# NVlabs/UnseenObjectClustering

Hardware: AMD Instinct MI355X
Metric: frames/sec at 640x480 RGB-D, two-stage clustering (higher is better)
Workload: dtype f32; 1 GPU; configs[3] frames: full two-stage (crop-and-refine) segmentation of single 640x480 RGB-D frames; throughput schedule 3 streams x 4-frame launch sets (one frame at a time: `latency`); frame=640x480, seeds=100, iters=10, crop=224, total_frames=513, frames_per_gpu=513, collective=False, frames_in_flight_per_gpu=12, streams_per_gpu=3, frames_per_launch=4

## Files before the change

### unseenobjectclustering_amd/csrc/meanshift.hip

```cpp
#include "common.h"
#include "prof.h"

#include <limits.h>
#include <math.h>
#include <stdlib.h>

#include <mutex>
#include <type_traits>
#include <utility>

namespace uoc {

constexpr int C = UOC_EMBED_DIM;
constexpr int FPS_THREADS = 256;
constexpr int FPS_MAX_BLOCKS = 1024;
constexpr int HC_THREADS = 256;
constexpr int HC_MAX_BLOCKS = 1024;
constexpr int ZP = 72;
constexpr int NLAB = UOC_MAX_SEEDS;

constexpr int MS_COSINE = UOC_METRIC_COSINE;
constexpr int MS_EUCLIDEAN = UOC_METRIC_EUCLIDEAN;
constexpr float XX_OUT = 1e30f;

struct ArgMax {
  float val;
  int idx;
};

__device__ __forceinline__ bool better(const ArgMax &a, const ArgMax &b) {
  return a.val > b.val || (a.val == b.val && a.idx < b.idx);
}

__device__ __forceinline__ ArgMax wave_argmax(ArgMax v) {
#pragma unroll
  for (int off = 32; off >= 1; off >>= 1) {
    ArgMax o;
    o.val = __shfl_xor(v.val, off);
    o.idx = __shfl_xor(v.idx, off);
    if (better(o, v)) v = o;
  }
  return v;
}

template <int NH, int MET>
__global__ __launch_bounds__(FPS_THREADS) void fps_step_kernel(
    const float *__restrict__ X, int n, int m, int step, int num_init, const int *__restrict__ first_index,
    float *__restrict__ dmin, float *__restrict__ seeds, int *__restrict__ indices,
    const ArgMax *__restrict__ part_in, ArgMax *__restrict__ part_out) {
  const int b = blockIdx.y;
  const int nblk = gridDim.x;
  X += (size_t)b * NH * n * C;
  dmin += (size_t)b * n;
  seeds += (size_t)b * NH * m * C;
  indices += (size_t)b * m;
  part_in += (size_t)b * FPS_MAX_BLOCKS;
  part_out += (size_t)b * FPS_MAX_BLOCKS;

  __shared__ ArgMax red[FPS_THREADS / 64];
  const int tid = threadIdx.x, lane = tid & 63, wave = tid >> 6;

  const bool given = step < num_init;
  int cur;
  if (given) {
    cur = -1;
  } else if (step == 0) {
    cur = first_index[b];
    if (cur < 0 || cur >= n) cur = 0;
  } else {
    ArgMax best = {-INFINITY, INT_MAX};
    for (int i = tid; i < nblk; i += FPS_THREADS) {
      ArgMax a = part_in[i];
      if (better(a, best)) best = a;
    }
    best = wave_argmax(best);
    if (lane == 0) red[wave] = best;
    __syncthreads();
    best = red[0];
#pragma unroll
    for (int w = 1; w < FPS_THREADS / 64; ++w)
      if (better(red[w], best)) best = red[w];
    cur = best.idx;
    if (cur < 0 || cur >= n) cur = 0;
    __syncthreads();
  }
  if (blockIdx.x == 0) {
    if (tid == 0) indices[step] = cur;
    if (!given && tid < NH * C)
      seeds[((size_t)(tid / C) * m + step) * C + tid % C] = X[((size_t)(tid / C) * n + cur) * C + tid % C];
  }
  if (step == m - 1) return;

  const int t = lane & 15, g = lane >> 4;
  float4 sv[NH];
#pragma unroll
  for (int h = 0; h < NH; ++h)
    sv[h] = given ? *reinterpret_cast<const float4 *>(seeds + ((size_t)h * m + step) * C + 4 * t)
                  : *reinterpret_cast<const float4 *>(X + ((size_t)h * n + cur) * C + 4 * t);
  ArgMax best = {-INFINITY, INT_MAX};
  const int nchunk = (n + 63) >> 6;
  for (int chunk = blockIdx.x * (FPS_THREADS / 64) + wave; chunk < nchunk; chunk += nblk * (FPS_THREADS / 64)) {
    const int base = chunk << 6;
    float4 x[NH][16];
#pragma unroll
    for (int h = 0; h < NH; ++h)
#pragma unroll
      for (int i = 0; i < 16; ++i) {
        const int p = base + 4 * i + g;
        x[h][i] = (p < n) ? *reinterpret_cast<const float4 *>(X + ((size_t)h * n + p) * C + 4 * t)
                          : make_float4(0.f, 0.f, 0.f, 0.f);
      }
    float mine = 0.f;
#pragma unroll
    for (int i = 0; i < 16; ++i) {
      float s;
      if constexpr (MET == MS_EUCLIDEAN) {
        s = 0.f;
#pragma unroll
        for (int h = 0; h < NH; ++h) {
          const float dx = x[h][i].x - sv[h].x, dy = x[h][i].y - sv[h].y, dz = x[h][i].z - sv[h].z,
                      dw = x[h][i].w - sv[h].w;
          s = fmaf(dx, dx, s);
          s = fmaf(dy, dy, s);
          s = fmaf(dz, dz, s);
          s = fmaf(dw, dw, s);
        }
      } else {
        s = x[0][i].x * sv[0].x;
        s = fmaf(x[0][i].y, sv[0].y, s);
        s = fmaf(x[0][i].z, sv[0].z, s);
        s = fmaf(x[0][i].w, sv[0].w, s);
#pragma unroll
        for (int h = 1; h < NH; ++h) {
          s = fmaf(x[h][i].x, sv[h].x, s);
          s = fmaf(x[h][i].y, sv[h].y, s);
          s = fmaf(x[h][i].z, sv[h].z, s);
          s = fmaf(x[h][i].w, sv[h].w, s);
        }
      }
      s = row16_sum(s);
      if (t == i) mine = s;
    }
    const int p = base + 4 * t + g;
    if (p < n) {
      float d = MET == MS_EUCLIDEAN ? sqrtf(mine) : 0.5f * (1.0f - mine);
      if (step > 0) d = fminf(d, dmin[p]);
      dmin[p] = d;
      if (d > best.val) {
        best.val = d;
        best.idx = p;
      }
    }
  }
  best = wave_argmax(best);
  if (lane == 0) red[wave] = best;
  __syncthreads();
  if (tid == 0) {
    best = red[0];
#pragma unroll
    for (int w = 1; w < FPS_THREADS / 64; ++w)
      if (better(red[w], best)) best = red[w];
    part_out[blockIdx.x] = best;
  }
}

__device__ int g_fps_timeout = 0;

constexpr int FPP_THREADS = 512;
constexpr int FPP_WAVES = FPP_THREADS / 64;
constexpr int FPP_RS = 3;
constexpr int FPP_LS = 1;
constexpr int FPP_SLOTS = FPP_RS + FPP_LS;
constexpr int FPP_PIX_PER_BLOCK = FPP_THREADS * FPP_SLOTS;

__device__ __forceinline__ ArgMax wave_argmax_fast(ArgMax a) {
  float v = a.val;
  v = fmaxf(v, dpp_f<0xB1>(v));
  v = fmaxf(v, dpp_f<0x4E>(v));
  v = fmaxf(v, dpp_f<0x141>(v));
  v = fmaxf(v, dpp_f<0x140>(v));
  const int vi = __float_as_int(v);
  const float m = fmaxf(fmaxf(__int_as_float(__builtin_amdgcn_readlane(vi, 0)), __int_as_float(__builtin_amdgcn_readlane(vi, 16))),
                        fmaxf(__int_as_float(__builtin_amdgcn_readlane(vi, 32)), __int_as_float(__builtin_amdgcn_readlane(vi, 48))));
  int i = (a.val == m) ? a.idx : INT_MAX;
  i = min(i, dpp_i<0xB1>(i));
  i = min(i, dpp_i<0x4E>(i));
  i = min(i, dpp_i<0x141>(i));
  i = min(i, dpp_i<0x140>(i));
  const int mi = min(min(__builtin_amdgcn_readlane(i, 0), __builtin_amdgcn_readlane(i, 16)),
                     min(__builtin_amdgcn_readlane(i, 32), __builtin_amdgcn_readlane(i, 48)));
  return ArgMax{m, mi};
}

__device__ __forceinline__ unsigned long long fpp_pack(float val, int idx, int tag) {
  return ((unsigned long long)__float_as_uint(val) << 32) | (unsigned)(idx & 0xFFFFFF) | ((unsigned)(tag & 0xFF) << 24);
}

template <int MET>
__global__ __launch_bounds__(FPP_THREADS) void fps_persistent_kernel(
    const float *__restrict__ X, int n, int m, int bpi, int nslots, const int *__restrict__ first_index,
    float *__restrict__ seeds, int *__restrict__ indices, unsigned long long *gran, int *status) {
  extern __shared__ __attribute__((aligned(16))) float smem[];
  __shared__ ArgMax red[FPP_WAVES];
  __shared__ int s_idx;
  const int item = blockIdx.x / bpi, blk = blockIdx.x - item * bpi;
  X += (size_t)item * n * C;
  seeds += (size_t)item * m * C;
  indices += (size_t)item * m;
  const int tid = threadIdx.x, lane = tid & 63, wave = tid >> 6;
  const int pbase = blk * (FPP_THREADS * nslots) + tid;
  float4 *lds = reinterpret_cast<float4 *>(smem) + tid;

  typedef float f32x2 __attribute__((ext_vector_type(2)));
  static_assert(FPP_RS == 3, "pixels 0/1 packed, pixel 2 scalar");
  f32x2 x01[C];
  float x2[C];
#pragma unroll
  for (int j = 0; j < FPP_RS; ++j) {
    const int p = pbase + j * FPP_THREADS;
    const bool ok = j < nslots && p < n;
#pragma unroll
    for (int c4 = 0; c4 < C / 4; ++c4) {
      const float4 v = ok ? *reinterpret_cast<const float4 *>(X + (size_t)p * C + 4 * c4) : make_float4(0.f, 0.f, 0.f, 0.f);
      const float e[4] = {v.x, v.y, v.z, v.w};
#pragma unroll
      for (int k = 0; k < 4; ++k) {
        if (j == 0) x01[4 * c4 + k].x = e[k];
        if (j == 1) x01[4 * c4 + k].y = e[k];
        if (j == 2) x2[4 * c4 + k] = e[k];
      }
    }
  }
  if (nslots > FPP_RS) {
    const int p = pbase + FPP_RS * FPP_THREADS;
#pragma unroll
    for (int c4 = 0; c4 < C / 4; ++c4)
      lds[c4 * FPP_THREADS] = (p < n) ? *reinterpret_cast<const float4 *>(X + (size_t)p * C + 4 * c4)
                                      : make_float4(0.f, 0.f, 0.f, 0.f);
  }
  float dm[FPP_SLOTS];
#pragma unroll
  for (int j = 0; j < FPP_SLOTS; ++j) dm[j] = 0.f;
  float xx[FPP_SLOTS] = {};
  if constexpr (MET == MS_EUCLIDEAN) {
    f32x2 q01 = {0.f, 0.f};
    float q2 = 0.f, q3 = 0.f;
#pragma unroll
    for (int c = 0; c < C; ++c) {
      q01 = __builtin_elementwise_fma(x01[c], x01[c], q01);
      q2 = fmaf(x2[c], x2[c], q2);
    }
    if (nslots > FPP_RS) {
#pragma unroll
      for (int c4 = 0; c4 < C / 4; ++c4) {
        const float4 v = lds[c4 * FPP_THREADS];
        q3 = fmaf(v.x, v.x, q3);
        q3 = fmaf(v.y, v.y, q3);
        q3 = fmaf(v.z, v.z, q3);
        q3 = fmaf(v.w, v.w, q3);
      }
    }
    xx[0] = q01.x;
    xx[1] = q01.y;
    xx[2] = q2;
    xx[3] = q3;
  }

  int cur = __builtin_amdgcn_readfirstlane(first_index[item]);
  if (cur < 0 || cur >= n) cur = 0;
  if (blk == 0) {
    if (tid == 0) indices[0] = cur;
    if (tid < 16) *reinterpret_cast<float4 *>(seeds + 4 * tid) = *reinterpret_cast<const float4 *>(X + (size_t)cur * C + 4 * tid);
  }
#ifdef UOC_FPS_TIMING
  unsigned long long tc_comp = 0, tc_red = 0, tc_sweep = 0, tc_tail = 0;
#define UOC_T(v) const unsigned long long v = __builtin_amdgcn_s_memtime()
#else
#define UOC_T(v)
#endif
  for (int step = 0; step + 1 < m; ++step) {
    UOC_T(t1_);
    const float *__restrict__ srow = X + (size_t)cur * C;
    ArgMax best = {-INFINITY, INT_MAX};
    f32x2 s01 = {0.f, 0.f};
#pragma unroll
    for (int c = 0; c < C; ++c) s01 = __builtin_elementwise_fma(x01[c], f32x2{srow[c], srow[c]}, s01);
    float ss = 0.f;
    if constexpr (MET == MS_EUCLIDEAN) {
#pragma unroll
      for (int c = 0; c < C; ++c) ss = fmaf(srow[c], srow[c], ss);
    }
    auto dist = [&](float s_, float xx_) {
      if constexpr (MET == MS_EUCLIDEAN) return sqrtf(fmaxf(fmaf(-2.0f, s_, xx_ + ss), 0.0f));
      else return 0.5f * (1.0f - s_);
    };
    float s2 = 0.f;
    if (nslots > 2) {
#pragma unroll
      for (int c = 0; c < C; ++c) s2 = fmaf(x2[c], srow[c], s2);
    }
#pragma unroll
    for (int j = 0; j < FPP_RS; ++j) {
      if (j < nslots) {
        const float s_ = j == 0 ? s01.x : j == 1 ? s01.y : s2;
        float d_ = dist(s_, xx[j]);
        if (step > 0) d_ = fminf(d_, dm[j]);
        dm[j] = d_;
        const int p_ = pbase + j * FPP_THREADS;
        if (p_ < n && d_ > best.val) {
          best.val = d_;
          best.idx = p_;
        }
      }
    }
    if (nslots > FPP_RS) {
      float s_ = 0.f;
#pragma unroll
      for (int c4 = 0; c4 < C / 4; ++c4) {
        const float4 v = lds[c4 * FPP_THREADS];
        s_ = fmaf(v.x, srow[4 * c4 + 0], s_);
        s_ = fmaf(v.y, srow[4 * c4 + 1], s_);
        s_ = fmaf(v.z, srow[4 * c4 + 2], s_);
        s_ = fmaf(v.w, srow[4 * c4 + 3], s_);
      }
      float d_ = dist(s_, xx[FPP_RS]);
      if (step > 0) d_ = fminf(d_, dm[FPP_RS]);
      dm[FPP_RS] = d_;
      const int p_ = pbase + FPP_RS * FPP_THREADS;
      if (p_ < n && d_ > best.val) {
        best.val = d_;
        best.idx = p_;
      }
    }
    UOC_T(t2_);
    best = wave_argmax_fast(best);
    if (lane == 0) red[wave] = best;
    __syncthreads();
    UOC_T(t3_);
    if (wave == 0) {
      ArgMax b2 = lane < FPP_WAVES ? red[lane] : ArgMax{-INFINITY, INT_MAX};
      b2 = wave_argmax_fast(b2);
      unsigned long long *row = gran + ((size_t)(step & 1) * gridDim.x + (size_t)item * bpi);
      const int tag = (step + 1) & 0xFF;
      if (lane == 0) __hip_atomic_store(row + blk, fpp_pack(b2.val, b2.idx, tag), __ATOMIC_RELAXED, __HIP_MEMORY_SCOPE_AGENT);
      ArgMax acc = {-INFINITY, INT_MAX};
      unsigned spins = 0;
      bool done = false;
      while (!done) {
        bool ok = true;
        ArgMax a = {-INFINITY, INT_MAX};
        unsigned long long gv[4];
#pragma unroll
        for (int k = 0; k < 4; ++k)
          gv[k] = (lane + 64 * k < bpi) ? __hip_atomic_load(row + lane + 64 * k, __ATOMIC_RELAXED, __HIP_MEMORY_SCOPE_AGENT)
                                        : ((unsigned long long)tag << 24);
#pragma unroll
        for (int k = 0; k < 4; ++k) {
          const unsigned long long v = gv[k];
          ok &= (int)((v >> 24) & 0xFF) == tag;
          if (lane + 64 * k < bpi) {
            ArgMax c = {__uint_as_float((unsigned)(v >> 32)), (int)(v & 0xFFFFFF)};
            if (better(c, a)) a = c;
          }
        }
        if (__all(ok)) {
          acc = a;
          done = true;
        } else {
          __builtin_amdgcn_s_sleep(1);
          if (++spins > (1u << 22) || (((spins & 1023) == 0) && __hip_atomic_load(status, __ATOMIC_RELAXED, __HIP_MEMORY_SCOPE_AGENT))) {
            if (lane == 0) {
              __hip_atomic_store(status, 1, __ATOMIC_RELAXED, __HIP_MEMORY_SCOPE_AGENT);
              __hip_atomic_store(&g_fps_timeout, 1, __ATOMIC_RELAXED, __HIP_MEMORY_SCOPE_AGENT);
            }
            acc = ArgMax{0.f, 0};
            done = true;
          }
        }
      }
      acc = wave_argmax_fast(acc);
      if (lane == 0) s_idx = acc.idx;
    }
    __syncthreads();
    UOC_T(t4_);
    cur = __builtin_amdgcn_readfirstlane(s_idx);
    if (cur < 0 || cur >= n) cur = 0;
    if (blk == 0) {
      if (tid == 0) indices[step + 1] = cur;
      if (tid < 16)
        *reinterpret_cast<float4 *>(seeds + (size_t)(step + 1) * C + 4 * tid) =
            *reinterpret_cast<const float4 *>(X + (size_t)cur * C + 4 * tid);
    }
#ifdef UOC_FPS_TIMING
    const unsigned long long t5_ = __builtin_amdgcn_s_memtime();
    tc_comp += t2_ - t1_;
    tc_red += t3_ - t2_;
    tc_sweep += t4_ - t3_;
    tc_tail += t5_ - t4_;
#endif
  }
#ifdef UOC_FPS_TIMING
  if ((blockIdx.x == 0 || blockIdx.x == gridDim.x / 2) && tid == 0)
    printf("[fps timing blk %d] per step (cycles): compute %.1f reduce %.1f sweep %.1f tail %.1f\n", (int)blockIdx.x,
           tc_comp / (double)(m - 1), tc_red / (double)(m - 1), tc_sweep / (double)(m - 1), tc_tail / (double)(m - 1));
#endif
#undef UOC_T
}

__device__ __forceinline__ float f4c(const float4 &v, int e) { return e == 0 ? v.x : e == 1 ? v.y : e == 2 ? v.z : v.w; }
__device__ __forceinline__ f32x4 mfma4(float a, float b, f32x4 c) {
  return __builtin_amdgcn_mfma_f32_16x16x4f32(a, b, c, 0, 0, 0);
}

template <int ST, int NH>
__device__ __forceinline__ void lds_stage_seeds(const float *Z, int m, int tid, float *Zs) {
  for (int i = tid; i < NH * ST * 16 * (C / 4); i += HC_THREADS) {
    const int h = i / (ST * 16 * (C / 4)), j = i % (ST * 16 * (C / 4));
    const int row = j / (C / 4), c4 = j % (C / 4);
    float4 v = make_float4(0.f, 0.f, 0.f, 0.f);
    if (row < m) v = *reinterpret_cast<const float4 *>(Z + ((size_t)h * m + row) * C + 4 * c4);
    *reinterpret_cast<float4 *>(Zs + (h * ST * 16 + row) * ZP + 4 * c4) = v;
  }
}
template <int ST, int NH>
__device__ __forceinline__ void lds_seed_norms(const float *Zs, int tid, float *zzs) {
  if (tid < ST * 16) {
    float p = 0.f;
    for (int h = 0; h < NH; ++h)
      for (int c = 0; c < C; ++c) {
        const float z = Zs[(h * ST * 16 + tid) * ZP + c];
        p = fmaf(z, z, p);
      }
    zzs[tid] = p;
  }
}
template <int NH>
__device__ __forceinline__ void lds_pixel_norms(const float4 (&xa)[NH * 4], int q, float (&xx)[4]) {
  float p = 0.f;
#pragma unroll
  for (int v = 0; v < NH * 4; ++v) {
    p = fmaf(xa[v].x, xa[v].x, p);
    p = fmaf(xa[v].y, xa[v].y, p);
    p = fmaf(xa[v].z, xa[v].z, p);
    p = fmaf(xa[v].w, xa[v].w, p);
  }
  p += __shfl_xor(p, 16);
  p += __shfl_xor(p, 32);
#pragma unroll
  for (int r = 0; r < 4; ++r) xx[r] = __shfl(p, 4 * q + r);
}

template <int ST, int NH, int MET>
__global__ __launch_bounds__(HC_THREADS) __attribute__((amdgpu_waves_per_eu(2))) void hc_iter_kernel(const float *__restrict__ X, int n,
                                                             const float *__restrict__ Z, int m, float kappa,
                                                             float *__restrict__ partial_, int nvb) {
  static_assert(NH == 2, "64-d fields run hc_iter_flat_kernel");
  extern __shared__ __attribute__((aligned(16))) float smem[];
  constexpr bool EUC = MET == MS_EUCLIDEAN;
  __shared__ float zzs[EUC ? ST * 16 : 1];
  __shared__ float wred[EUC ? 4 * ST * 16 : 1];
  float *Zs = smem;
  const int b = blockIdx.y;
  const int nblk = nvb;
  const int hz = blockIdx.z;
  X += (size_t)b * NH * n * C;
  Z += (size_t)b * NH * m * C;

  const int tid = threadIdx.x, lane = tid & 63, wave = tid >> 6;
  const int t = lane & 15, q = lane >> 4;
  float *const wpartial = partial_ + (size_t)gridDim.y * nblk * NH * (ST * 16) * C;
  for (int vb = blockIdx.x; vb < nvb; vb += gridDim.x) {
  float *partial = partial_ + (((size_t)b * nblk + vb) * NH + hz) * (ST * 16) * C;

  lds_stage_seeds<ST, NH>(Z, m, tid, Zs);
  __syncthreads();
  float ws[ST];
  if constexpr (EUC) {
    lds_seed_norms<ST, NH>(Zs, tid, zzs);
#pragma unroll
    for (int s = 0; s < ST; ++s) ws[s] = 0.f;
    __syncthreads();
  }

  f32x4 acc[ST][4];
#pragma unroll
  for (int s = 0; s < ST; ++s)
#pragma unroll
    for (int ct = 0; ct < 4; ++ct) acc[s][ct] = f32x4{0.f, 0.f, 0.f, 0.f};

  const int ntile = (n + 15) >> 4;
  const int stride = nblk * (HC_THREADS / 64);
  int tile = vb * (HC_THREADS / 64) + wave;

  float4 xa[NH * 4], xb[4];
  auto load_tile = [&](int tl, float4(&a)[NH * 4], float4(&bb)[4]) {
    const int pa = tl * 16 + t;
#pragma unroll
    for (int v = 0; v < NH * 4; ++v)
      a[v] = (tl < ntile && pa < n)
                 ? *reinterpret_cast<const float4 *>(X + ((size_t)(v >> 2) * n + pa) * C + 16 * (v & 3) + 4 * q)
                 : make_float4(0.f, 0.f, 0.f, 0.f);
#pragma unroll
    for (int r = 0; r < 4; ++r) {
      const int pb = tl * 16 + 4 * q + r;
      bb[r] = (tl < ntile && pb < n) ? *reinterpret_cast<const float4 *>(X + ((size_t)hz * n + pb) * C + 4 * t)
                                     : make_float4(0.f, 0.f, 0.f, 0.f);
    }
  };
  load_tile(tile, xa, xb);

  for (; tile < ntile; tile += stride) {
    f32x4 Sv[ST];
    float wv[ST][4];
    int zo = 0;
    asm volatile("" : "+v"(zo));
    const float *Zt = Zs + zo;
    float xx[4];
    if constexpr (EUC) {
      lds_pixel_norms<NH>(xa, q, xx);
#pragma unroll
      for (int r = 0; r < 4; ++r)
        if (tile * 16 + 4 * q + r >= n) xx[r] = XX_OUT;
    }
#pragma unroll
    for (int i = 0; i < ST + 2; ++i) {
      if (i >= 1 && i - 1 < ST) {
        if constexpr (EUC) {
          const float zz = zzs[16 * (i - 1) + t];
#pragma unroll
          for (int r = 0; r < 4; ++r)
            wv[i - 1][r] = expf(-kappa * fmaxf(fmaf(-2.0f, Sv[i - 1][r], zz + xx[r]), 0.0f));
          ws[i - 1] += (wv[i - 1][0] + wv[i - 1][1]) + (wv[i - 1][2] + wv[i - 1][3]);
        } else {
#pragma unroll
          for (int r = 0; r < 4; ++r) wv[i - 1][r] = expf(kappa * Sv[i - 1][r]);
        }
      }
      if (i < ST) Sv[i] = f32x4{0.f, 0.f, 0.f, 0.f};
      if (i < ST) {
#pragma unroll
        for (int k = 0; k < 16; ++k) {
          const int v = k >> 2, e = k & 3;
          const float4 zb = *reinterpret_cast<const float4 *>(Zt + (ST * 16 + 16 * i + t) * ZP + 16 * v + 4 * q);
          Sv[i] = mfma4(f4c(xa[4 + v], e), f4c(zb, e), Sv[i]);
        }
      }
#pragma unroll
      for (int k = 0; k < 16; ++k) {
        if (i < ST) {
          const int v = k >> 2, e = k & 3;
          const float4 zb = *reinterpret_cast<const float4 *>(Zt + (16 * i + t) * ZP + 16 * v + 4 * q);
          Sv[i] = mfma4(f4c(xa[v], e), f4c(zb, e), Sv[i]);
        }
        if (i >= 2) {
          const int r = k >> 2, ct = k & 3;
          acc[i - 2][ct] = mfma4(wv[i - 2][r], f4c(xb[r], ct), acc[i - 2][ct]);
        }
      }
    }
// ... 949 lines not shown
  ArgMax *part[2];
  float *hc_partial;
  int *counts;
  int *num_unique;
  int *seed_labels;
  float *Z;
  int hc_nblk;
  int nh;
  size_t total;
};

static int hc_virtual_blocks(int n) {
  const int ntile = (n + 15) / 16;
  const int tiles_per_wave = 16;
  int nvb = (ntile + 4 * tiles_per_wave - 1) / (4 * tiles_per_wave);
  if (nvb > 256) nvb = 256;
  if (nvb < 1) nvb = 1;
  return nvb;
}

static int hc_physical_blocks(int batch, int nvb, int per_cu) {
  const int slots = (device_num_cu() > 0 ? device_num_cu() : 256) * per_cu;
  int best = 1;
  long best_cost = -1;
  for (int p = 1; p <= nvb; ++p) {
    const long rounds = ((long)p * batch + slots - 1) / slots;
    const long cost = rounds * ((nvb + p - 1) / p);
    if (best_cost < 0 || cost < best_cost) {
      best_cost = cost;
      best = p;
    }
  }
  return best;
}

static int hc_blocks(int batch, int n) {
  const int ntile = (n + 15) / 16;
  int nblk = 512 / (batch > 0 ? batch : 1);
  if (nblk < 8) nblk = 8;
  const int maxb = (ntile + 3) / 4;
  if (nblk > maxb) nblk = maxb;
  if (nblk > HC_MAX_BLOCKS) nblk = HC_MAX_BLOCKS;
  if (nblk < 1) nblk = 1;
  return nblk;
}

static MsWorkspace carve(void *base, int batch, int n, int nh = 1) {
  MsWorkspace w;
  size_t off = 0;
  auto take = [&](size_t bytes) {
    void *p = base ? (void *)((char *)base + off) : nullptr;
    off += align_up(bytes, 256);
    return p;
  };
  w.hc_nblk = hc_virtual_blocks(n);
  w.dmin = (float *)take((size_t)batch * n * sizeof(float));
  w.part[0] = (ArgMax *)take((size_t)batch * FPS_MAX_BLOCKS * sizeof(ArgMax));
  w.part[1] = (ArgMax *)take((size_t)batch * FPS_MAX_BLOCKS * sizeof(ArgMax));
  w.hc_partial = (float *)take((size_t)batch * w.hc_nblk * (nh * NLAB * C + NLAB) * sizeof(float));
  w.counts = (int *)take((size_t)batch * NLAB * sizeof(int));
  w.num_unique = (int *)take((size_t)batch * sizeof(int));
  w.seed_labels = (int *)take((size_t)batch * NLAB * sizeof(int));
  w.Z = (float *)take((size_t)batch * nh * NLAB * C * sizeof(float));
  w.nh = nh;
  w.total = off;
  return w;
}

static int check_common(const void *X, int batch, int n, int m, void *ws, size_t ws_bytes, int nh = 1) {
  UOC_REQUIRE(X != nullptr, "X is null");
  UOC_REQUIRE(batch >= 1 && batch <= 65535, "batch=%d out of range [1,65535]", batch);
  UOC_REQUIRE(n >= 1, "n=%d must be >= 1", n);
  UOC_REQUIRE(m >= 1 && m <= UOC_MAX_SEEDS, "num_seeds=%d out of range [1,%d]", m, UOC_MAX_SEEDS);
  UOC_REQUIRE(((uintptr_t)X & 15) == 0, "X must be 16-byte aligned");
  const size_t need = carve(nullptr, batch, n, nh).total;
  UOC_REQUIRE(ws != nullptr && ws_bytes >= need, "workspace too small: %zu < %zu", ws_bytes, need);
  UOC_REQUIRE(((uintptr_t)ws & 255) == 0, "workspace must be 256-byte aligned");
  return UOC_OK;
}

static int fps_blocks(int n) {
  const int nchunk = (n + 63) / 64;
  int nblk = (nchunk + 3) / 4;
  if (nblk > FPS_MAX_BLOCKS) nblk = FPS_MAX_BLOCKS;
  if (nblk < 1) nblk = 1;
  return nblk;
}

static int g_fps_persistent = -1;
static std::atomic<int> g_fps_fallbacks{0};
static std::atomic<int> g_fps_stream_ordering{0};
static int fps_persistent_plan(int batch, int n, int *bpi, int *nslots) {
  const int g_num_cu = device_num_cu();
  if (g_num_cu <= 0) return 0;
  if (g_fps_persistent < 0) {
    const char *e = getenv("UOC_FPS_PERSISTENT");
    g_fps_persistent = e ? atoi(e) : 1;
  }
  if (!g_fps_persistent || n >= (1 << 24)) return 0;
  int b = g_num_cu / batch;
  if (b < 1) return 0;
  if (b > 256) b = 256;
  const int per_block = (n + b - 1) / b;
  int ns = (per_block + FPP_THREADS - 1) / FPP_THREADS;
  if (ns > FPP_SLOTS) return 0;
  if (ns < 1) ns = 1;
  const int pack = FPP_SLOTS;
  if (pack > ns) ns = pack < FPP_SLOTS ? pack : FPP_SLOTS;
  b = (n + FPP_THREADS * ns - 1) / (FPP_THREADS * ns);
  *bpi = b;
  *nslots = ns;
  return 1;
}

template <int... Vs, class F>
static void dispatch(int v, F &&f) {
  (void)((v == Vs && (f(std::integral_constant<int, Vs>{}), true)) || ...);
}
template <class F>
static void dispatch_metric_halves(int met, int nh, F &&f) {
  dispatch<MS_COSINE, MS_EUCLIDEAN>(met, [&](auto MET) { dispatch<1, 2>(nh, [&](auto NH) { f(MET, NH); }); });
}
template <class F>
static void dispatch_shape(int met, int nh, int m, F &&f) {
  dispatch_metric_halves(met, nh, [&](auto MET, auto NH) {
    dispatch<1, 2, 3, 4, 5, 6, 7, 8>((m + 15) / 16, [&](auto ST) { f(ST, NH, MET); });
  });
}

static int run_select_seeds_streaming(const float *X, int batch, int n, int m, const int32_t *first, float *seeds,
                                      int32_t *indices, const MsWorkspace &w, hipStream_t st, int num_init = 0,
                                      int met = MS_COSINE);

struct FpsChain {
  std::mutex mu;
  hipEvent_t ev[kMaxDevices] = {};
  hipEvent_t event() {
    const int d = current_device();
    if (!ev[d] && hipEventCreateWithFlags(&ev[d], hipEventDisableTiming) != hipSuccess) ev[d] = nullptr;
    return ev[d];
  }
};
static FpsChain &fps_chain() {
  static FpsChain *c = new FpsChain();
  return *c;
}

static int run_select_seeds(const float *X, int batch, int n, int m, const int32_t *first, float *seeds,
                            int32_t *indices, const MsWorkspace &w, hipStream_t st, int met = MS_COSINE) {
  const void *fpp = nullptr;
  dispatch<MS_COSINE, MS_EUCLIDEAN>(met,
                                    [&](auto MET) { fpp = reinterpret_cast<const void *>(&fps_persistent_kernel<MET>); });
  int done = 0;
  while (m >= 2 && done < batch && w.nh == 1) {
    int sub = batch - done, bpi = 0, nslots = 0;
    while (sub > 1 && !fps_persistent_plan(sub, n, &bpi, &nslots)) --sub;
    if (!fps_persistent_plan(sub, n, &bpi, &nslots)) break;
    const int launches = (batch - done + sub - 1) / sub;
    sub = (batch - done + launches - 1) / launches;
    if (!fps_persistent_plan(sub, n, &bpi, &nslots)) break;
    unsigned long long *gran = reinterpret_cast<unsigned long long *>(w.part[0]);
    const size_t gbytes = (size_t)2 * sub * bpi * sizeof(unsigned long long);
    if (gbytes + sizeof(unsigned long long) > (size_t)batch * FPS_MAX_BLOCKS * sizeof(ArgMax)) break;
    int *status = reinterpret_cast<int *>(gran + (size_t)2 * sub * bpi);
    UOC_HIP_CHECK(hipMemsetAsync(gran, 0, gbytes + sizeof(unsigned long long), st));
    const size_t lds = (nslots > FPP_RS) ? (size_t)FPP_LS * (C / 4) * FPP_THREADS * sizeof(float4) : 0;
    static DeviceOnce attr_set[2];
    if (!attr_set[met].done()) {
      UOC_HIP_CHECK(hipFuncSetAttribute(fpp, hipFuncAttributeMaxDynamicSharedMemorySize,
                                        (int)((size_t)FPP_LS * (C / 4) * FPP_THREADS * sizeof(float4))));
      attr_set[met].mark();
    }
    const float *Xc = X + (size_t)done * n * C;
    const int32_t *fc = first + done;
    float *sc = seeds + (size_t)done * m * C;
    int32_t *ic = indices + (size_t)done * m;
    void *args[] = {(void *)&Xc, (void *)&n, (void *)&m, (void *)&bpi, (void *)&nslots, (void *)&fc,
                    (void *)&sc, (void *)&ic, (void *)&gran, (void *)&status};
    hipError_t e;
    {
      FpsChain &chain = fps_chain();
      std::lock_guard<std::mutex> lock(chain.mu);
      const bool capturing = stream_is_capturing(st);
      hipEvent_t ev = (g_fps_stream_ordering.load() && !capturing) ? chain.event() : nullptr;
      if (ev) UOC_HIP_CHECK(hipStreamWaitEvent(st, ev, 0));
      {
        ProfScope prof(KC_FPS_STEP, st, 2.0 * sub * (double)n * C * (m - 1), 4.0 * sub * (double)n * C,
                       ProfTag{{n, sub, bpi, nslots}});
        if (!capturing)
          e = hipLaunchCooperativeKernel(fpp, dim3(sub * bpi), dim3(FPP_THREADS), args, (unsigned)lds, st);
        else
          e = hipLaunchKernel(fpp, dim3(sub * bpi), dim3(FPP_THREADS), args, lds, st);
      }
      if (e == hipSuccess && ev) UOC_HIP_CHECK(hipEventRecord(ev, st));
    }
    if (e != hipSuccess) {
      (void)hipGetLastError();
      break;
    }
    done += sub;
  }
  if (done >= batch) return UOC_OK;
  if (g_fps_persistent != 0 && w.nh == 1 && m >= 2) {
    if (g_fps_fallbacks.fetch_add(1) == 0)
      fprintf(stderr, "[uoc] farthest-point sampling: %d of %d field(s) of n=%d ran on the streaming kernel (the on-chip "
              "kernel does not fit / is not co-resident on this device); see uoc_ms_fps_fallbacks()\n", batch - done, batch, n);
  }
  return run_select_seeds_streaming(X + (size_t)done * w.nh * n * C, batch - done, n, m, first + done,
                                    seeds + (size_t)done * w.nh * m * C, indices + (size_t)done * m, w, st, 0, met);
}

static int run_select_seeds_streaming(const float *X, int batch, int n, int m, const int32_t *first, float *seeds,
                                      int32_t *indices, const MsWorkspace &w, hipStream_t st, int num_init, int met) {
  const int nblk = fps_blocks(n);
  dispatch_metric_halves(met, w.nh, [&](auto MET, auto NH) {
    for (int s = 0; s < m; ++s) {
      dim3 grid(nblk, batch);
      const bool last = s == m - 1;
      ProfScope prof(KC_FPS_STEP, st, last ? 0.0 : 2.0 * batch * n * C * w.nh,
                     last ? 0.0 : 4.0 * batch * ((double)n * C * w.nh + 2.0 * n));
      hipLaunchKernelGGL((fps_step_kernel<NH, MET>), grid, dim3(FPS_THREADS), 0, st, X, n, m, s, num_init, first, w.dmin,
                         seeds, indices, w.part[(s + 1) & 1], w.part[s & 1]);
    }
  });
  UOC_LAUNCH_CHECK();
  return UOC_OK;
}

constexpr double HC_COST_TILES = 6.1;
constexpr double HC_COST_ITEM = 0.76;
constexpr double HC_COST_NEXT = 0.3;
static double hc_part_cost(int P, int p) {
  const double tiles = P == 2 ? (p == 0 ? 3.1 : 3.0) : P == 3 ? (p == 0 ? 2.1 : 2.0) : (p == 0 ? 1.1 : 1.0);
  return tiles + HC_COST_ITEM;
}
static double hc_plan_cost(const HcPlan &p) {
  double phase1 = 0.0;
  if (p.n1 > 0) {
    const int c = (p.n1 + p.grid - 1) / p.grid;
    phase1 = c * HC_COST_TILES + HC_COST_ITEM + (c - 1) * HC_COST_NEXT;
  }
  const int R = p.items - p.n1, T = R * p.parts;
  double tail = 0.0;
  for (int g = 0; g < p.grid && T > 0; ++g) {
    double c = 0.0;
    for (int k = 0; k < 2; ++k) {
      const int t = k * p.grid + ((k & 1) ? p.grid - 1 - g : g);
      if (t < T) c += hc_part_cost(p.parts, t / R);
    }
    if (c > tail) tail = c;
  }
  return phase1 + tail;
}
static EnvInt g_hc_parts("UOC_HC_PARTS", 0);
static HcPlan hc_make_plan(int batch, int nvb, bool splittable) {
  const int cus = device_num_cu() > 0 ? device_num_cu() : 256;
  HcPlan whole;
  whole.nvb = nvb;
  whole.items = batch * nvb;
  whole.n1 = whole.items;
  whole.parts = 1;
  whole.grid = whole.items < cus ? whole.items : cus;
  if (!splittable) return whole;
  const int force = g_hc_parts.get();
  if (force == 1) return whole;
  HcPlan best = whole;
  double best_cost = hc_plan_cost(whole);
  static const int cand[3] = {2, 3, 6};
  for (int ci = 0; ci < 3; ++ci) {
    const int P = cand[ci];
    if (force > 1 && force != P) continue;
    const int q = whole.items / cus;
    for (int back = 0; back <= 1; ++back) {
      if (q - back < 0) break;
      HcPlan c = whole;
      c.parts = P;
      c.n1 = (q - back) * cus;
      const int T = (c.items - c.n1) * P;
      if (T == 0) continue;
      c.grid = c.n1 > 0 ? cus : (T < cus ? T : cus);
      if (T > 2 * c.grid) continue;
      const double cost = hc_plan_cost(c);
      if (force > 1 ? (best.parts != P || cost < best_cost) : cost < 0.985 * best_cost) {
        best = c;
        best_cost = cost;
      }
    }
  }
  return best;
}

template <int ST, int NH, int MET>
static void launch_hc(const float *X, int batch, int n, float *Z, int m, float kappa, int iters,
                      const MsWorkspace &w, hipStream_t st) {
  const int nvb = w.hc_nblk;
  const int last = m - 16 * (ST - 1);
  const bool quad = ST >= 2 && last >= 1 && last <= 4;
  HcPlan plan = {};
  int phys;
  size_t lds;
  if constexpr (NH == 1) {
    plan = hc_make_plan(batch, nvb, ST == 7 && quad);
    phys = plan.grid;
    lds = (size_t)4 * ST * 4 * 64 * sizeof(f32x4) + (MET == MS_EUCLIDEAN ? (size_t)4 * ST * 16 * sizeof(float) : 0);
    static DeviceOnce attr_set;
    if (!attr_set.done() && lds > 64 * 1024) {
      (void)hipFuncSetAttribute(reinterpret_cast<const void *>(&hc_iter_flat_kernel<ST, false, MET>),
                                hipFuncAttributeMaxDynamicSharedMemorySize, (int)lds);
      if constexpr (ST >= 2)
        (void)hipFuncSetAttribute(reinterpret_cast<const void *>(&hc_iter_flat_kernel<ST, true, MET>),
                                  hipFuncAttributeMaxDynamicSharedMemorySize, (int)lds);
      attr_set.mark();
    }
  } else {
    phys = hc_physical_blocks(batch, nvb, 2);
    const size_t zbytes = (size_t)NH * ST * 16 * ZP * sizeof(float);
    const size_t rbytes = (size_t)2 * ST * 4 * 64 * sizeof(f32x4);
    lds = zbytes > rbytes ? zbytes : rbytes;
    static DeviceOnce attr_set;
// ... 327 lines not shown
```

Measured before the change: 174.7 frames/s.

## Pipeline FPS seed-row loads in chunks and defer seed writeback to kernel end

The per-step distance computation in the persistent farthest-point-sampling kernel now runs in four 16-channel chunks. The next chunk's seed row and LDS pixel data are fetched while FMAs on the current chunk run, with the LDS slot's dot product done via inline scalar-operand v_fmac. Selected indices are kept in an LDS list, and all seed rows and indices are written once at the end instead of by block 0 every step. The winning row is also touched in wave 0 right after the reduction to warm the cache. The cost is manual scheduling barriers and inline asm that constrain the compiler, a hard limit on num_seeds, and LDS that is now always allocated.

```diff
diff --git a/unseenobjectclustering_amd/csrc/meanshift.hip b/unseenobjectclustering_amd/csrc/meanshift.hip
--- a/unseenobjectclustering_amd/csrc/meanshift.hip
+++ b/unseenobjectclustering_amd/csrc/meanshift.hip
@@ -172,6 +172,9 @@
 constexpr int FPP_LS = 1;
 constexpr int FPP_SLOTS = FPP_RS + FPP_LS;
 constexpr int FPP_PIX_PER_BLOCK = FPP_THREADS * FPP_SLOTS;
+constexpr int FPP_CH = 16;
+constexpr int FPP_NCH = C / FPP_CH;
+constexpr int FPP_MAX_M = UOC_MAX_SEEDS;
 
 __device__ __forceinline__ ArgMax wave_argmax_fast(ArgMax a) {
   float v = a.val;
@@ -203,6 +206,7 @@
   extern __shared__ __attribute__((aligned(16))) float smem[];
   __shared__ ArgMax red[FPP_WAVES];
   __shared__ int s_idx;
+  __shared__ int s_list[FPP_MAX_M];
   const int item = blockIdx.x / bpi, blk = blockIdx.x - item * bpi;
   X += (size_t)item * n * C;
   seeds += (size_t)item * m * C;
@@ -219,24 +223,27 @@
   for (int j = 0; j < FPP_RS; ++j) {
     const int p = pbase + j * FPP_THREADS;
     const bool ok = j < nslots && p < n;
+    const float *src = X + (size_t)(ok ? p : 0) * C;
 #pragma unroll
     for (int c4 = 0; c4 < C / 4; ++c4) {
-      const float4 v = ok ? *reinterpret_cast<const float4 *>(X + (size_t)p * C + 4 * c4) : make_float4(0.f, 0.f, 0.f, 0.f);
+      const float4 v = *reinterpret_cast<const float4 *>(src + 4 * c4);
       const float e[4] = {v.x, v.y, v.z, v.w};
 #pragma unroll
       for (int k = 0; k < 4; ++k) {
-        if (j == 0) x01[4 * c4 + k].x = e[k];
-        if (j == 1) x01[4 * c4 + k].y = e[k];
-        if (j == 2) x2[4 * c4 + k] = e[k];
+        if (j == 0) x01[4 * c4 + k].x = ok ? e[k] : 0.f;
+        if (j == 1) x01[4 * c4 + k].y = ok ? e[k] : 0.f;
+        if (j == 2) x2[4 * c4 + k] = ok ? e[k] : 0.f;
       }
     }
   }
   if (nslots > FPP_RS) {
     const int p = pbase + FPP_RS * FPP_THREADS;
-#pragma unroll
-    for (int c4 = 0; c4 < C / 4; ++c4)
-      lds[c4 * FPP_THREADS] = (p < n) ? *reinterpret_cast<const float4 *>(X + (size_t)p * C + 4 * c4)
-                                      : make_float4(0.f, 0.f, 0.f, 0.f);
+    const float *src = X + (size_t)(p < n ? p : 0) * C;
+#pragma unroll
+    for (int c4 = 0; c4 < C / 4; ++c4) {
+      const float4 v = *reinterpret_cast<const float4 *>(src + 4 * c4);
+      lds[c4 * FPP_THREADS] = (p < n) ? v : make_float4(0.f, 0.f, 0.f, 0.f);
+    }
   }
   float dm[FPP_SLOTS];
 #pragma unroll
@@ -268,37 +275,82 @@
 
   int cur = __builtin_amdgcn_readfirstlane(first_index[item]);
   if (cur < 0 || cur >= n) cur = 0;
-  if (blk == 0) {
-    if (tid == 0) indices[0] = cur;
-    if (tid < 16) *reinterpret_cast<float4 *>(seeds + 4 * tid) = *reinterpret_cast<const float4 *>(X + (size_t)cur * C + 4 * tid);
-  }
+  if (tid == 0) s_list[0] = cur;
 #ifdef UOC_FPS_TIMING
-  unsigned long long tc_comp = 0, tc_red = 0, tc_sweep = 0, tc_tail = 0;
-#define UOC_T(v) const unsigned long long v = __builtin_amdgcn_s_memtime()
+  unsigned long long tc_[6] = {0, 0, 0, 0, 0, 0}, t1p_ = 0, t5p_ = 0;
+#define UOC_T(v)                                                                    \
+  unsigned long long v;                                                             \
+  __builtin_amdgcn_sched_barrier(0);                                                \
+  asm volatile("s_memtime %0\n\ts_waitcnt lgkmcnt(0)" : "=s"(v) : : "memory");     \
+  __builtin_amdgcn_sched_barrier(0)
+  UOC_T(tbegin_);
 #else
 #define UOC_T(v)
 #endif
+  float pf = 0.f;
+  __builtin_amdgcn_s_waitcnt(0x0F70);
   for (int step = 0; step + 1 < m; ++step) {
-    UOC_T(t1_);
+    UOC_T(t0_);
+#ifdef UOC_FPS_TIMING
+    if (step > 0) tc_[5] += t0_ - t5p_;
+#endif
     const float *__restrict__ srow = X + (size_t)cur * C;
     ArgMax best = {-INFINITY, INT_MAX};
     f32x2 s01 = {0.f, 0.f};
-#pragma unroll
-    for (int c = 0; c < C; ++c) s01 = __builtin_elementwise_fma(x01[c], f32x2{srow[c], srow[c]}, s01);
-    float ss = 0.f;
-    if constexpr (MET == MS_EUCLIDEAN) {
-#pragma unroll
-      for (int c = 0; c < C; ++c) ss = fmaf(srow[c], srow[c], ss);
+    float s2 = 0.f, s3 = 0.f, ss = 0.f;
+    {
+      float r[FPP_NCH][FPP_CH];
+      float4 l[FPP_NCH][FPP_CH / 4];
+      auto fetch_row = [&](int k) {
+#pragma unroll
+        for (int c = 0; c < FPP_CH; ++c) r[k][c] = srow[k * FPP_CH + c];
+      };
+      auto fetch_lds = [&](int k) {
+#pragma unroll
+        for (int q = 0; q < FPP_CH / 4; ++q) l[k][q] = lds[(k * (FPP_CH / 4) + q) * FPP_THREADS];
+      };
+      auto fmac4 = [](float &acc, const float *sc, const float4 &v) {
+        asm("v_fmac_f32 %0, %1, %5\n\tv_fmac_f32 %0, %2, %6\n\tv_fmac_f32 %0, %3, %7\n\tv_fmac_f32 %0, %4, %8"
+            : "+v"(acc)
+            : "s"(sc[0]), "s"(sc[1]), "s"(sc[2]), "s"(sc[3]), "v"(v.x), "v"(v.y), "v"(v.z), "v"(v.w));
+      };
+      fetch_row(0);
+      fetch_lds(0);
+#pragma unroll
+      for (int k = 0; k < FPP_NCH; ++k) {
+        __builtin_amdgcn_sched_barrier(0);
+        __builtin_amdgcn_s_waitcnt(0xC07F);
+        __builtin_amdgcn_sched_barrier(0);
+#ifdef UOC_FPS_TIMING
+        if (k == 0) {
+          UOC_T(t1_);
+          tc_[0] += t1_ - t0_;
+          t1p_ = t1_;
+        }
+#endif
+        if (k + 1 < FPP_NCH) fetch_row(k + 1);
+        __builtin_amdgcn_sched_barrier(0);
+#pragma unroll
+        for (int q = 0; q < FPP_CH / 4; ++q) fmac4(s3, &r[k][4 * q], l[k][q]);
+        __builtin_amdgcn_sched_barrier(0);
+        if (k + 1 < FPP_NCH) fetch_lds(k + 1);
+        __builtin_amdgcn_sched_barrier(0);
+#pragma unroll
+        for (int c = 0; c < FPP_CH; ++c) s01 = __builtin_elementwise_fma(x01[k * FPP_CH + c], f32x2{r[k][c], r[k][c]}, s01);
+        if constexpr (MET == MS_EUCLIDEAN) {
+#pragma unroll
+          for (int c = 0; c < FPP_CH; ++c) ss = fmaf(r[k][c], r[k][c], ss);
+        }
+        if (nslots > 2) {
+#pragma unroll
+          for (int c = 0; c < FPP_CH; ++c) s2 = fmaf(x2[k * FPP_CH + c], r[k][c], s2);
+        }
+      }
     }
     auto dist = [&](float s_, float xx_) {
       if constexpr (MET == MS_EUCLIDEAN) return sqrtf(fmaxf(fmaf(-2.0f, s_, xx_ + ss), 0.0f));
       else return 0.5f * (1.0f - s_);
     };
-    float s2 = 0.f;
-    if (nslots > 2) {
-#pragma unroll
-      for (int c = 0; c < C; ++c) s2 = fmaf(x2[c], srow[c], s2);
-    }
 #pragma unroll
     for (int j = 0; j < FPP_RS; ++j) {
       if (j < nslots) {
@@ -314,16 +366,7 @@
       }
     }
     if (nslots > FPP_RS) {
-      float s_ = 0.f;
-#pragma unroll
-      for (int c4 = 0; c4 < C / 4; ++c4) {
-        const float4 v = lds[c4 * FPP_THREADS];
-        s_ = fmaf(v.x, srow[4 * c4 + 0], s_);
-        s_ = fmaf(v.y, srow[4 * c4 + 1], s_);
-        s_ = fmaf(v.z, srow[4 * c4 + 2], s_);
-        s_ = fmaf(v.w, srow[4 * c4 + 3], s_);
-      }
-      float d_ = dist(s_, xx[FPP_RS]);
+      float d_ = dist(s3, xx[FPP_RS]);
       if (step > 0) d_ = fminf(d_, dm[FPP_RS]);
       dm[FPP_RS] = d_;
       const int p_ = pbase + FPP_RS * FPP_THREADS;
@@ -336,13 +379,15 @@
     best = wave_argmax_fast(best);
     if (lane == 0) red[wave] = best;
     __syncthreads();
-    UOC_T(t3_);
     if (wave == 0) {
+      asm volatile("" : : "v"(pf));
       ArgMax b2 = lane < FPP_WAVES ? red[lane] : ArgMax{-INFINITY, INT_MAX};
       b2 = wave_argmax_fast(b2);
+      UOC_T(t3_);
       unsigned long long *row = gran + ((size_t)(step & 1) * gridDim.x + (size_t)item * bpi);
       const int tag = (step + 1) & 0xFF;
       if (lane == 0) __hip_atomic_store(row + blk, fpp_pack(b2.val, b2.idx, tag), __ATOMIC_RELAXED, __HIP_MEMORY_SCOPE_AGENT);
+      UOC_T(t4_);
       ArgMax acc = {-INFINITY, INT_MAX};
       unsigned spins = 0;
       bool done = false;
@@ -378,33 +423,52 @@
           }
         }
       }
+      UOC_T(t5_);
       acc = wave_argmax_fast(acc);
+      int w = acc.idx;
+      if (w < 0 || w >= n) w = 0;
+      pf = X[(size_t)w * C + lane];
       if (lane == 0) s_idx = acc.idx;
+#ifdef UOC_FPS_TIMING
+      tc_[1] += t2_ - t1p_;
+      tc_[2] += t3_ - t2_;
+      tc_[3] += t4_ - t3_;
+      tc_[4] += t5_ - t4_;
+      t5p_ = t5_;
+#endif
     }
     __syncthreads();
-    UOC_T(t4_);
     cur = __builtin_amdgcn_readfirstlane(s_idx);
     if (cur < 0 || cur >= n) cur = 0;
-    if (blk == 0) {
-      if (tid == 0) indices[step + 1] = cur;
-      if (tid < 16)
-        *reinterpret_cast<float4 *>(seeds + (size_t)(step + 1) * C + 4 * tid) =
-            *reinterpret_cast<const float4 *>(X + (size_t)cur * C + 4 * tid);
-    }
+    if (tid == 0) s_list[step + 1] = cur;
+  }
 #ifdef UOC_FPS_TIMING
-    const unsigned long long t5_ = __builtin_amdgcn_s_memtime();
-    tc_comp += t2_ - t1_;
-    tc_red += t3_ - t2_;
-    tc_sweep += t4_ - t3_;
-    tc_tail += t5_ - t4_;
-#endif
-  }
-#ifdef UOC_FPS_TIMING
-  if ((blockIdx.x == 0 || blockIdx.x == gridDim.x / 2) && tid == 0)
-    printf("[fps timing blk %d] per step (cycles): compute %.1f reduce %.1f sweep %.1f tail %.1f\n", (int)blockIdx.x,
-           tc_comp / (double)(m - 1), tc_red / (double)(m - 1), tc_sweep / (double)(m - 1), tc_tail / (double)(m - 1));
+  {
+    UOC_T(tend_);
+    if (m > 1) tc_[5] += tend_ - t5p_;
+    if (tid == 0)
+      printf("[fps timing] n %d bpi %d item %d blk %d steps %d total %llu : row %llu fma %llu reduce %llu publish %llu seen %llu handoff %llu\n",
+             n, bpi, item, blk, m - 1, tend_ - tbegin_, tc_[0], tc_[1], tc_[2], tc_[3], tc_[4], tc_[5]);
+  }
 #endif
 #undef UOC_T
+  if (blk == 0) {
+    __syncthreads();
+    for (int i = tid; i < m; i += FPP_THREADS) indices[i] = s_list[i];
+    static_assert(FPP_MAX_M * (C / 4) <= 4 * FPP_THREADS, "four 16-byte pieces per thread cover every seed row");
+    float4 v[4];
+#pragma unroll
+    for (int u = 0; u < 4; ++u) {
+      const int q = tid + u * FPP_THREADS;
+      v[u] = make_float4(0.f, 0.f, 0.f, 0.f);
+      if (q < m * (C / 4)) v[u] =*reinterpret_cast<const float4 *>(X + (size_t)s_list[q >> 4] * C + 4 * (q & 15));
+    }
+#pragma unroll
+    for (int u = 0; u < 4; ++u) {
+      const int q = tid + u * FPP_THREADS;
+      if (q < m * (C / 4)) *reinterpret_cast<float4 *>(seeds + (size_t)(q >> 4) * C + 4 * (q & 15)) = v[u];
+    }
+  }
 }
 
 __device__ __forceinline__ float f4c(const float4 &v, int e) { return e == 0 ? v.x : e == 1 ? v.y : e == 2 ? v.z : v.w; }
@@ -1660,6 +1724,7 @@
   dispatch<MS_COSINE, MS_EUCLIDEAN>(met,
                                     [&](auto MET) { fpp = reinterpret_cast<const void *>(&fps_persistent_kernel<MET>); });
   int done = 0;
+  UOC_REQUIRE(m <= FPP_MAX_M, "num_seeds=%d exceeds the on-chip index list (%d)", m, FPP_MAX_M);
   while (m >= 2 && done < batch && w.nh == 1) {
     int sub = batch - done, bpi = 0, nslots = 0;
     while (sub > 1 && !fps_persistent_plan(sub, n, &bpi, &nslots)) --sub;
@@ -1672,7 +1737,7 @@
     if (gbytes + sizeof(unsigned long long) > (size_t)batch * FPS_MAX_BLOCKS * sizeof(ArgMax)) break;
     int *status = reinterpret_cast<int *>(gran + (size_t)2 * sub * bpi);
     UOC_HIP_CHECK(hipMemsetAsync(gran, 0, gbytes + sizeof(unsigned long long), st));
-    const size_t lds = (nslots > FPP_RS) ? (size_t)FPP_LS * (C / 4) * FPP_THREADS * sizeof(float4) : 0;
+    const size_t lds = (size_t)FPP_LS * (C / 4) * FPP_THREADS * sizeof(float4);
     static DeviceOnce attr_set[2];
     if (!attr_set[met].done()) {
       UOC_HIP_CHECK(hipFuncSetAttribute(fpp, hipFuncAttributeMaxDynamicSharedMemorySize,
```

After: 176.0 frames/s, median of 6. Within noise of the previous version (+0.8%).
